# NathanBWaters/playaid_core

Measured on AMD Instinct MI355X. Metric: 1080p frames/sec end-to-end, higher is better.
Workload: dtype f32; 1 GPU; configs[1]: 64 x 1080x1920 BGR frames per GPU per clip; parallelism=single GPU, lanes=2, ingest=raw BGR frames resident in HBM

## Files before the change

include/playaid_hip.h:

```cpp
#ifndef PLAYAID_HIP_H
#define PLAYAID_HIP_H

#include <stddef.h>
#include <stdint.h>

#ifdef __cplusplus
extern "C" {
#endif

#define PA_ABI_VERSION 15
#define PA_WEIGHT_MAGIC 0x31574150
#define PA_LSTM_MAGIC 0x314c4150
#define PA_ENCODER_MAGIC 0x31454150
#define PA_FEATURE_STRIDE 1024
#define PA_CROP 128

typedef enum pa_status {
    PA_OK = 0,
    PA_ERR_INVALID_ARG = -1,
    PA_ERR_HIP = -2,
    PA_ERR_BAD_WEIGHTS = -3,
    PA_ERR_CAPACITY = -4,
    PA_ERR_NO_DEVICE = -5,
    PA_ERR_NOT_READY = -6,
// ... 312 lines not shown
int pa_wino_transform_weights(const float* w_host, int32_t cin, int32_t cout, int32_t bn, float* ug_host);
int pa_wino_conv3x3(const float* x, const float* ug, const float* bias, const float* residual, float* out, int32_t n,
                    int32_t height, int32_t width, int32_t cin, int32_t cout, int32_t bn, int32_t in_px_stride,
                    int32_t out_px_stride, int32_t out_pad, int32_t act, int32_t res_after, void* stream);
int pa_wino_conv3x3_splitk(const float* x, const float* ug, const float* bias, const float* residual, float* out, int32_t n,
                           int32_t height, int32_t width, int32_t cin, int32_t cout, int32_t bn, int32_t in_px_stride, int32_t out_px_stride,
                           int32_t out_pad, int32_t act, int32_t res_after, float* slab, size_t slab_floats, int32_t* tickets,
                           int32_t n_tickets, void* stream);

size_t pa_conv_weight_bytes(int32_t cin, int32_t cout, int32_t ksize, int32_t compute_dtype, int32_t has_residual);
int pa_conv_pack_weights(const float* w_host, int32_t cin, int32_t cout, int32_t ksize, int32_t compute_dtype, int32_t has_residual,
                         void* out_host);
int pa_conv2d(const float* x, const void* w, const float* bias, const float* residual, float* out, int32_t n, int32_t height,
              int32_t width, int32_t cin, int32_t cout, int32_t ksize, int32_t stride, int32_t in_pad, int32_t in_px_stride,
              int32_t out_px_stride, int32_t out_pad, int32_t act, int32_t res_after, int32_t compute_dtype, void* stream);

typedef struct pa_encoder pa_encoder;
size_t pa_encoder_blob_bytes(int32_t in_dim, int32_t hidden_dim, int32_t slots, int32_t enc_dim, int32_t num_layers,
                             int32_t ff_dim, int32_t num_actions);
int pa_encoder_create(int32_t device, int32_t in_dim, int32_t hidden_dim, int32_t slots, int32_t enc_dim, int32_t num_heads,
                      int32_t num_layers, int32_t ff_dim, int32_t num_actions, int32_t max_rows, const void* blob_host,
                      size_t blob_bytes, pa_encoder** out);
void pa_encoder_destroy(pa_encoder* h);
const char* pa_encoder_last_error(const pa_encoder* h);
int pa_encoder_forward(pa_encoder* h, const float* feats, int32_t ld, int32_t seq_len, int32_t batch, float* logp, void* stream);


int pa_profile_enable(pa_engine* e, int32_t on);
int pa_profile_read(pa_engine* e, pa_kernel_stat* stats, int32_t max_stats, int32_t* n_stats);

// ... 48 lines not shown
```

playaid_core_amd/_lib.py:

```python
from __future__ import annotations

import ctypes as C
import os

HERE = os.path.dirname(os.path.abspath(__file__))
LIB_PATH = os.environ.get("PA_LIB_PATH") or os.path.join(HERE, "libplayaid_hip.so")

PA_ABI_VERSION = 15
PA_DTYPE_F32 = 0
PA_DTYPE_BF16 = 1
PA_DTYPE_EMULATED_F32 = 2
DTYPES = {"f32": PA_DTYPE_F32, "bf16": PA_DTYPE_BF16, "emulated_f32": PA_DTYPE_EMULATED_F32}
PA_WEIGHT_MAGIC = 0x31574150
PA_LSTM_MAGIC = 0x314C4150
PA_ENCODER_MAGIC = 0x31454150
PA_FEATURE_STRIDE = 1024
PA_TRACE_STAGES = 20
DET_FORMS = ("not_run", "stem_direct", "stem_bf16", "wino", "patch", "pgemm", "pgemm_up", "psgemm", "psgemm_up", "igemm", "sppf",
             "maxpool", "upsample", "absorbed", "decode", "bgemm", "bgemm_up")
CN_FORMS = ("not_run", "stem_pool", "avgpool", "wino", "patch", "igemm_128x128", "igemm_128x64", "igemm_64x64", "psgemm",
            "bgemm", "bgemm_splitk", "avgpool_bf16")
LSTM_FORMS = ("not_run", "steps", "u1", "u2", "u4", "u8", "mfma")

PA_OK = 0
# ... 165 lines not shown
    ("pa_convnet_destroy", None, [_P]),
    ("pa_convnet_last_error", C.c_char_p, [_P]),
    ("pa_convnet_forward", C.c_int, [_P, _P, C.c_int32, _P, C.c_int32, _P]),
    ("pa_convnet_trace", C.c_int, [_P, _P, C.c_int32, C.c_int32, C.c_int32, _P, C.c_size_t, _P]),
    ("pa_convnet_layer_forms", C.c_int, [_P, _P, C.c_int32]),
    ("pa_detector_plan", C.c_int, [_P] * 5 + [C.c_int32] + [_P] * 7),
    ("pa_detector_plan_desc", C.c_int, [_P, _P, _P, C.c_int32, C.c_int32, C.c_longlong, _P, C.c_int32, C.c_longlong, _P]),
    ("pa_square_crops_src", C.c_int, [_P, _P, C.c_int32, C.c_int32, C.c_int32, _P, _P, C.c_int32, C.c_int32, C.c_int32, _P, _P, _P]),
    ("pa_wino_weight_floats", C.c_size_t, [C.c_int32, C.c_int32]),
    ("pa_wino_channels_per_workgroup", C.c_int, [C.c_int32, C.c_int64]),
    ("pa_wino_transform_weights", C.c_int, [_P, C.c_int32, C.c_int32, C.c_int32, _P]),
    ("pa_wino_conv3x3", C.c_int, [_P, _P, _P, _P, _P] + [C.c_int32] * 11 + [_P]),
    ("pa_conv_weight_bytes", C.c_size_t, [C.c_int32] * 5),
    ("pa_conv_pack_weights", C.c_int, [_P] + [C.c_int32] * 5 + [_P]),
    ("pa_conv2d", C.c_int, [_P, _P, _P, _P, _P] + [C.c_int32] * 14 + [_P]),
    ("pa_wino_conv3x3_splitk", C.c_int, [_P, _P, _P, _P, _P] + [C.c_int32] * 11 + [_P, C.c_size_t, _P, C.c_int32, _P]),
    ("pa_crop_resize_width", C.c_int, [_P, _P, C.c_int32, C.c_int32, C.c_int32, C.POINTER(C.c_int32), C.c_int32, C.c_int32, _P, C.c_int32,
                                       C.POINTER(C.c_int32), _P]),
    ("pa_encoder_blob_bytes", C.c_size_t, [C.c_int32] * 7),
    ("pa_encoder_create", C.c_int, [C.c_int32] * 10 + [_P, C.c_size_t, C.POINTER(_P)]),
    ("pa_encoder_destroy", None, [_P]),
    ("pa_encoder_last_error", C.c_char_p, [_P]),
    ("pa_encoder_forward", C.c_int, [_P, _P, C.c_int32, C.c_int32, C.c_int32, _P, _P]),
    ("pa_mjpeg_create", C.c_int, [C.c_int32, C.c_int32, C.c_int32, C.c_int32, C.c_size_t, C.POINTER(_P)]),
    ("pa_mjpeg_destroy", None, [_P]),
    ("pa_mjpeg_last_error", C.c_char_p, [_P]),
    ("pa_mjpeg_probe", C.c_int, [_P, C.c_size_t, C.POINTER(C.c_int32), C.c_char_p, C.c_size_t]),
    ("pa_mjpeg_set_sync_rounds", C.c_int, [_P, C.c_int32]),
    ("pa_mjpeg_set_groups", C.c_int, [_P, C.c_int32]),
    ("pa_mjpeg_last_sync_rounds", C.c_int, [_P]),
# ... 56 lines not shown
```

playaid_core_amd/conv.py:

```python
from __future__ import annotations

import ctypes as C

import numpy as np
import torch

from . import _lib


def pack_weights(w_oihw: np.ndarray, compute_dtype: str = "emulated_f32", has_residual: bool = False) -> np.ndarray:
    lib = _lib.load()
    w = np.ascontiguousarray(np.asarray(w_oihw, dtype=np.float32).transpose(0, 2, 3, 1))
    cout, k, _, cin = w.shape
    dt = _lib.DTYPES[compute_dtype]
    nbytes = lib.pa_conv_weight_bytes(cin, cout, k, dt, int(has_residual))
    if nbytes == 0:
        raise ValueError("cin and cout must be multiples of 32, the kernel 1x1 or 3x3, the dtype 'f32' or 'emulated_f32'")
    out = np.empty(nbytes, dtype=np.uint8)
    rc = lib.pa_conv_pack_weights(w.ctypes.data_as(C.c_void_p), cin, cout, k, dt, int(has_residual), out.ctypes.data_as(C.c_void_p))
    if rc:
        raise ValueError(f"pa_conv_pack_weights: status {rc}")
    return out


# ... 5 lines not shown
        raise ValueError("x_pad: contiguous float32[n, H + 2 pad, W + 2 pad, C] on the device")
    in_pad = (ksize - 1) // 2 if in_pad is None else in_pad
    n, hp, wp, cs = x_pad.shape
    h, w = hp - 2 * in_pad, wp - 2 * in_pad
    oh, ow = h // stride, w // stride
    ops = out_px_stride or cout
    if out is None:
        out = torch.zeros((n, oh + 2 * out_pad, ow + 2 * out_pad, ops), dtype=torch.float32, device=x_pad.device)
    ptr = lambda t_: C.c_void_p(t_.data_ptr()) if t_ is not None else C.c_void_p(0)
    stream = C.c_void_p(torch.cuda.current_stream(x_pad.device).cuda_stream)
    rc = lib.pa_conv2d(ptr(x_pad), ptr(w_packed), ptr(bias), ptr(residual), ptr(out), n, h, w, cin, cout, ksize, stride, in_pad, cs, out.shape[3],
                       out_pad, int(act), int(bool(res_after)), _lib.DTYPES[compute_dtype], stream)
    if rc:
        raise ValueError(f"pa_conv2d: status {rc}")
    return out
```

playaid_core_amd/csrc/conv_rows.hip:

```cpp
#include "conv_rows.h"
#include "../../include/playaid_hip.h"

namespace pa {

GemmParams conv_row_params(const ConvRow& r) {
    const int oh = r.in_h / r.stride, ow = r.in_w / r.stride;
    const int in_hb = r.in_h + 2 * r.in_pad, in_wb = r.in_w + 2 * r.in_pad;
    const int out_hb = oh + 2 * r.out_pad, out_wb = ow + 2 * r.out_pad;
    GemmParams p;
    memset(&p, 0, sizeof(p));
    p.M = r.images * oh * ow;
    p.N = r.cout;
    p.taps = r.ksize * r.ksize;
    p.kw_taps = r.ksize;
    p.chunk = r.cin;
    p.ktot = p.taps * p.chunk;
    p.howo = oh * ow;
    p.wo = ow;
    p.in_px_stride = r.in_px_stride;
    p.in_row_stride = in_wb * r.in_px_stride;
    p.in_img_stride = in_hb * in_wb * r.in_px_stride;
    p.stride = r.stride;
    p.off_y = p.off_x = r.in_pad - (r.ksize - 1) / 2;
    p.out_px_stride = r.out_px_stride;
// ... 119 lines not shown
    if ((long long)n * in_hb * in_wb * in_px_stride >= (1ll << 29) || (long long)n * out_hb * out_wb * out_px_stride >= (1ll << 29)) return PA_ERR_CAPACITY;
    pa::GemmParams p = pa::conv_row_params({ n,  height, width, in_pad, in_px_stride,  cin, cout, ksize, stride,
                                             out_pad, out_px_stride,  act, res_after});
    p.act = x;
    p.wgt = static_cast<const float*>(w);
    p.bias = bias;
    p.residual = residual;
    p.out = out;
    hipError_t e;
    if (compute_dtype == PA_DTYPE_EMULATED_F32) e = pa::launch_psgemm(p, static_cast<const unsigned short*>(w), (size_t)n * p.out_img_stride, 0, static_cast<hipStream_t>(stream));
    else if (residual) return PA_ERR_INVALID_ARG;
    else e = pa::launch_pgemm(p, 0, static_cast<hipStream_t>(stream));
    return e == hipSuccess ? PA_OK : (e == hipErrorInvalidValue ? PA_ERR_INVALID_ARG : PA_ERR_HIP);
}

}
```

playaid_core_amd/csrc/pa_api.hip:

```cpp
#include "../../include/playaid_hip.h"
#include "conv_rows.h"

#include <algorithm>
#include <cmath>
#include <cstdio>
#include <cstdlib>
#include <cstring>
#include <string>
#include <vector>

using namespace pa;

namespace {

constexpr int WINO_TICKETS = 4096;

struct ConvLayer {
    std::string name;
    int cin, cout, kh, kw, stride;
    int in_hw, out_hw;
    int in_pad, out_pad;
    int off;
    int taps, kw_taps, chunk;
    int in_px_stride;
// ... 2 lines not shown
    float* residual = nullptr;
    float* wgt = nullptr;
    float* wino_wgt = nullptr;
    int wino_bn = 0;
    float* bias = nullptr;
    int relu = 1;
    GemmTile tile = TILE_128x64;
    int splitk = 1;
    bool forced = false;
    float* in2 = nullptr;
    int in2_c = 0, in2_hw = 0, in2_stride = 1;
    float* ds_wgt = nullptr;
    float* ds_out = nullptr;
    float* ds_next_wgt = nullptr;
    float* ds_next_out = nullptr;
    bool ds_fused = false;
    bool ds_probe = false;
    double k_alg = 0;
    unsigned short* split_wgt = nullptr;
    unsigned short* ds_split_wgt = nullptr;
};

struct ProfEntry {
    int name_id;
    hipEvent_t start, stop;
    double flops, bytes;
    double flops_executed;
};

}
// ... 274 lines not shown
    p.ktot = L.taps * L.chunk;
    p.skip_w = L.kh == 7;
    p.howo = L.out_hw * L.out_hw;
    p.wo = L.out_hw;
    p.in_px_stride = L.in_px_stride;
    p.in_row_stride = in_w * L.in_px_stride;
    p.in_img_stride = (int)in_crop;
    p.stride = L.stride;
    p.off_y = L.off;
    p.off_x = L.off;
    p.out_px_stride = L.cout;
    p.out_row_stride = out_w * L.cout;
    p.out_img_stride = (int)out_crop;
    p.out_pad = L.out_pad;
    p.relu = L.relu;
    auto branch_gemm = [&]() {
        GemmParams d = conv_row_params({ ncrops,  L.in2_hw, L.in2_hw, 1, L.in2_c,
                                         L.in2_c, L.cout, 1, L.in2_stride,
                                         L.out_pad, L.cout,  0, 0});
        d.act = at(L.in2, (size_t)crop0 * (L.in2_hw + 2) * (L.in2_hw + 2) * L.in2_c);
        d.wgt = L.ds_wgt;
        d.out = at(L.ds_out, crop0 * out_crop);
        d.slab = p.slab;
        return d;
    };
    if (bf_ds && L.ds_fused) {
        p.residual = at(L.ds_out, crop0 * out_crop);
    } else if (bf_ds) {
        const GemmParams d = branch_gemm();
        ProfScope ps(e, s, prof_name, 2.0 * d.M * d.N * L.in2_c,
                     2.0 * ((double)ncrops * L.in2_hw * L.in2_hw * L.in2_c / (L.in2_stride * L.in2_stride) + (double)d.M * d.N + (double)d.N * L.in2_c));
        HIPCHK(e, launch_igemm_bf16(d, TILE_128x64, s));
        p.residual = d.out;
    } else if (f32_ds) {
        const GemmParams d = branch_gemm();
        ProfScope ps(e, s, prof_name, ds_done ? 0.0 : 2.0 * d.M * d.N * L.in2_c,
                     ds_done ? 0.0 : 4.0 * ((double)ncrops * L.in2_hw * L.in2_hw * L.in2_c / (L.in2_stride * L.in2_stride) + (double)d.M * d.N + (double)d.N * L.in2_c));
        if (ds_done) {
        } else if (e->emu && L.ds_split_wgt) {
            HIPCHK(e, launch_psgemm(d, L.ds_split_wgt, (size_t)ncrops * out_crop, 0, s));
        } else {
            GemmTile dt;
            int dsk;
            choose_tile(d.M, d.N, L.in2_c / 32, &dt, &dsk);
            HIPCHK(e, launch_igemm(d, dt, s));
        }
        if (ds_only) return PA_OK;
        p.residual = d.out;
    } else if (L.in2) {
        const int w2 = L.in2_hw + 2;
        p.act2 = at(L.in2, (size_t)crop0 * w2 * w2 * L.in2_c);
        p.k2_steps = L.in2_c / (bf ? 64 : 32);
        p.in2_px_stride = L.in2_c;
        p.in2_row_stride = w2 * L.in2_c;
        p.in2_img_stride = w2 * w2 * L.in2_c;
        p.stride2 = L.in2_stride;
        p.off2 = 1;
        p.ktot += L.in2_c;
    }
    GemmTile tile = L.tile;
    int splitk = L.splitk;
    if (!L.forced) choose_tile(p.M, p.N, p.ktot / (bf ? 64 : 32), &tile, &splitk);
    p.splitk = splitk;
    const size_t slab_avail = e->slab_floats > slab_off ? e->slab_floats - slab_off : 0;
    if ((size_t)p.splitk * p.M * p.N > slab_avail) p.splitk = 1;
    const bool ds_here = bf && L.ds_next_wgt;
    if (ds_here) {
        p.wgt2 = L.ds_next_wgt;
        p.out2 = at(L.ds_next_out, crop0 * out_crop);
    }
    if (ds_here || (bf && L.ds_probe)) {
        tile = (p.N % 128 == 0 && ((p.M + 127) / 128) * (p.N / 128) >= 256) ? TILE_128x128 : TILE_128x64;
        p.splitk = 1;
    }
    const double k_main = ((bf_ds || f32_ds) ? L.k_alg - L.in2_c : L.k_alg) + (ds_here ? L.cin : 0);
    const double flops = 2.0 * p.M * p.N * k_main;
    const double bytes = (double)es * ((double)ncrops * L.in_hw * L.in_hw * L.cin + (double)p.M * p.N * ((L.residual || bf_ds || f32_ds || ds_here) ? 2 : 1) +
                                       (double)p.N * k_main + ((L.in2 && !bf_ds && !f32_ds) ? (double)ncrops * L.in2_hw * L.in2_hw * L.in2_c : 0.0));
    const bool as_wino = !bf && L.wino_wgt && !p.act2;
    ProfScope ps(e, s, prof_name, flops, bytes, as_wino ? flops * 4.0 / 9.0 : flops);
    static const int use_patch = getenv("PA_PATCH") ? atoi(getenv("PA_PATCH")) : 1;
    static const int use_bf16_patch = getenv("PA_BF16_PATCH") ? atoi(getenv("PA_BF16_PATCH")) : 1;
    if (e->emu && L.split_wgt && !p.act2 && !p.residual) {
        HIPCHK(e, launch_psgemm(p, L.split_wgt, (size_t)ncrops * out_crop, 0, s));
    } else if (bf) {
        hipError_t pe = hipErrorInvalidValue;
        if (use_bf16_patch && L.stride == 1 && !p.act2) pe = launch_conv3x3_bf16_patch(p, s);
        if (pe == hipErrorInvalidValue) {
            static const int t256 = getenv("PA_BF16_T256") ? atoi(getenv("PA_BF16_T256")) : 1;
            if (t256 && !p.out2 && tile == TILE_128x128 && p.splitk == 1 && ((p.M + 255) / 256) * (p.N / 128) >= 256) tile = TILE_256x128;
            pe = launch_igemm_bf16(p, tile, s);
        }
        HIPCHK(e, pe);
    } else if (L.wino_wgt && !p.act2) {
        WinoParams q = wino_params(p, ncrops, L.out_hw, L.out_hw, L.cin, L.wino_wgt, L.wino_bn);
        if (e->wino_tickets && e->slab) {
            q.slab = e->slab + slab_off;
            q.slab_floats = e->slab_floats > slab_off ? std::min(e->slab_floats - slab_off, e->slab_floats / 2) : 0;
            q.tickets = reinterpret_cast<int32_t*>(e->wino_tickets) + (slab_off ? WINO_TICKETS : 0);
            q.tickets_cap = WINO_TICKETS;
        }
        HIPCHK(e, launch_wino3x3(q, s));
    } else if (use_patch && L.kh == 3 && L.stride == 1) {
        int bm = tile == TILE_64x64 || tile == TILE_64x64_K64 ? 64 : 128;
        const int howo = L.out_hw * L.out_hw, in_w2 = L.out_hw + 2;
        const int px128 = howo >= 128 ? (128 / L.out_hw + 2) * in_w2 : (128 / howo) * in_w2 * in_w2;
        if (bm == 128 && px128 > 224) bm = 64;
        hipError_t pe = launch_conv3x3_patch(p, bm, s);
        if (pe == hipErrorInvalidValue) pe = launch_igemm(p, tile, s);
        HIPCHK(e, pe);
    } else {
        static const int use_pgemm = getenv("PA_S2_PGEMM") ? atoi(getenv("PA_S2_PGEMM")) : 2;
        hipError_t pe = hipErrorInvalidValue;
        if (use_pgemm && L.kh == 3 && L.stride == 2 && !p.act2 && !p.residual && p.splitk <= 1 && !p.gather) pe = launch_pgemm(p, use_pgemm == 2 ? 64 : 0, s);
        if (pe == hipErrorInvalidValue) pe = launch_igemm(p, tile, s);
        HIPCHK(e, pe);
    }
    return PA_OK;
}

int run_backbone_part(pa_engine* e, int crop0, int ncrops, const float* x_in, float* feats_out, size_t slab_off, hipStream_t s,
                      int stop = PA_TRACE_STAGES) {
    int rc;
    ConvLayer stem = e->convs[0];
    stem.in = const_cast<float*>(x_in);
    static const bool stem_igemm = getenv("PA_STEM_IGEMM") && atoi(getenv("PA_STEM_IGEMM"));
    auto stem_part = [&](int c0, int n, hipStream_t st) -> int {
        if (stem_igemm && !e->bf16) return run_conv(e, stem, c0, n, slab_off, st, "igemm_conv7x7_stem");
        StemParams sp;
        memset(&sp, 0, sizeof(sp));
        sp.x = x_in + (size_t)c0 * 134 * 134 * 4;
// ... 436 lines not shown
                    rc = upload(e, &L.wgt, wf);
                    if (rc) return rc;
                    static const int wino_mode = getenv("PA_WINO") ? atoi(getenv("PA_WINO")) : 1;
                    static const int wino_ds = getenv("PA_WINO_DS") ? atoi(getenv("PA_WINO_DS")) : 1;
                    static const int wino_min_hw = getenv("PA_WINO_MIN_HW") ? atoi(getenv("PA_WINO_MIN_HW")) : 4;
                    if (wino_mode && wino_ds && hw_out >= wino_min_hw && hw_out % 4 == 0) {
                        L.wino_bn = wino_pick_bn(co, (long long)NC * (hw_out / 4) * (hw_out / 4), co);
                        std::vector<float> ug(wino_weight_floats(co, co), 0.f);
                        if (!br.dry) wino_transform_weights(keep_w.data(), co, co, L.wino_bn, ug.data());
                        rc = upload(e, &L.wino_wgt, ug);
                        if (rc) return rc;
                        rc = upload(e, &L.ds_wgt, wd);
                        if (rc) return rc;
                        if (e->emu && (rc = upload_split(e, &L.ds_split_wgt, wd, co, cin, false))) return rc;
                        ALLOC(L.ds_out, buf, true);
                    }
                }
                rc = upload(e, &L.bias, bf);
                if (rc) return rc;
                L.in2 = cur;
                L.in2_c = cin;
                L.in2_hw = hw_in[li];
                L.in2_stride = stride;
                L.k_alg += cin;
            }
            rc = add_conv(pre + ".1.conv1", co, co, 3, 1, hw_out, outA, mid, nullptr, 1);
            if (rc) return rc;
            rc = add_conv(pre + ".1.conv2", co, co, 3, 1, hw_out, mid, outB, outA, 1);
            if (rc) return rc;
            cur = outB;
// ... 999 lines not shown
```

playaid_core_amd/csrc/pigemm.hip:

```cpp
#include "pgemm_common.h"

#include <algorithm>
#include <type_traits>
#include <cstdio>
#include <cstdlib>
#include <vector>

namespace pa {


namespace {

typedef __attribute__((address_space(3))) float lds_f32;
typedef __attribute__((address_space(3))) f32x4 lds_f32x4;

template <int N> __device__ __forceinline__ void pg_wait_vm() { wait_vmcnt<(N > 63 ? 63 : N)>(); }

}

template <int BM, int BN = 64, bool SILU = true, bool STAMP = false, bool UP = false>
__global__ __launch_bounds__(256, 2) void pgemm_kernel(const GemmParams p) {
    auto stamp = [&](int i) {
        if (STAMP) {
            const unsigned long long t = __builtin_amdgcn_s_memtime();
            if ((threadIdx.x & 63) == 0) p.clk[((size_t)blockIdx.x * 4 + (threadIdx.x >> 6)) * 64 + i] = t;
        }
    };
    stamp(0);
    constexpr int WM = BN == 64 ? 2 : 4;
    constexpr int MI = BM / WM / 32;
    constexpr int A_ROWS = BM / 32, B_ROWS = BN / 32;
    constexpr int NLD = A_ROWS + B_ROWS;
    constexpr int NST = MI * 4 * (UP ? 5 : 1);
    constexpr int STAGE = (BM + BN) * 32;
    __shared__ __attribute__((aligned(16))) float lds[3 * STAGE];

    const TileRun run = tile_run(p);
    const int tile_n = run.tile_n, nt = run.nt;
    {
        const float *pa_ = p.act, *pw_ = p.wgt, *pb_ = p.bias;
        float* po_ = p.out;
        const int i0 = p.M, i1 = p.ktot, i2 = p.kw_taps, i3 = p.chunk, i4 = p.howo, i5 = p.wo, i6 = p.in_img_stride, i7 = p.in_row_stride,
                  i8 = p.in_px_stride, i9 = p.stride, i10 = p.off_y, i11 = p.off_x, i12 = p.out_img_stride, i13 = p.out_row_stride,
                  i14 = p.out_px_stride, i15 = p.out_pad, i16 = p.pg_ho, i17 = p.pg_nwx, i18 = p.pg_nwy;
        const unsigned u0 = p.pg_magic_howo, u1 = p.pg_magic_wo;
        asm volatile("" ::"s"(pa_), "s"(pw_), "s"(pb_), "s"(po_), "s"(i0), "s"(i1), "s"(i2), "s"(i3), "s"(i4), "s"(i5), "s"(i6), "s"(i7), "s"(i8), "s"(i9),
                     "s"(i10), "s"(i11), "s"(i12), "s"(i13), "s"(i14), "s"(i15), "s"(i16), "s"(i17), "s"(i18), "s"(u0), "s"(u1));
    }
    if (nt == 0) return;
    stamp(60);
    const int nk = p.ktot >> 5;
    const int total = nt * nk;

    const int tid = threadIdx.x;
    const int wave_id = __builtin_amdgcn_readfirstlane(tid >> 6);
    const int row0 = tid >> 3;
    const int colq = (tid & 7) ^ ((row0 >> 1) & 7);
    const int lane = tid & 63, lr = lane & 31, lh = lane >> 5;
    const int wm = BN == 64 ? wave_id >> 1 : wave_id, wn = BN == 64 ? wave_id & 1 : 0;

    const __amdgpu_buffer_rsrc_t act_rs = glds_rsrc(p.act), wgt_rs = glds_rsrc(p.wgt);

    const int ch0 = tile_n * BN + wn * 32 + 4 * lh;
    f32x2 nl2e = f32x2{-1.44269504088896341f, -1.44269504088896341f}, one2 = f32x2{1.f, 1.f};
    asm volatile("" : "+v"(nl2e), "+v"(one2));

    int b_off[B_ROWS];
#pragma unroll
    for (int i = 0; i < B_ROWS; ++i) b_off[i] = ((tile_n * BN + row0 + 32 * i) * p.ktot + colq * 4) * 4;

    const int in_ps = p.in_px_stride * p.stride * 4, in_rs = p.in_row_stride * p.stride * 4;
    const int in_wrap_x = in_rs - p.wo * in_ps;
    const int in_wrap_y = p.in_img_stride * 4 - p.pg_ho * in_rs;
    const int in_org = (p.off_y * p.in_row_stride + p.off_x * p.in_px_stride) * 4;
    int in_lane = row0 * in_ps + colq * 16;
    asm volatile("" : "+v"(in_lane));
    const PixelGeom geom = pixel_geom(p);
    int in_last;
    {
        int oy, ox;
        in_last = pixel_base(geom, p.M - 1, p.in_img_stride * 4, in_rs, in_ps, oy, ox) + in_org + colq * 16;
    }
    auto in_offset = [&](int m_base) {
        const int off = pixel_walk(geom, m_base, row0, p.in_img_stride * 4, in_rs, in_ps, in_wrap_x, in_wrap_y, in_org + in_lane);
// ... 13 lines not shown
    auto rows_of = [&](int tile_m) {
#pragma unroll
        for (int i = 0; i < A_ROWS; ++i) a_off[i] = in_offset(tile_m * BM + 32 * i);
    };
    rows_of(cur.tile);
    stamp(61);
    auto issue = [&](int slot) {
        float* As_w = lds + slot * STAGE + wave_id * 256;
        float* Bs_w = As_w + BM * 32;
        const int tapoff = cur.tap_offset(p) * 4;
#pragma unroll
        for (int i = 0; i < A_ROWS; ++i) glds16(act_rs, a_off[i], tapoff, As_w + i * 1024);
        const int koff = ((cur.ky * p.kw_taps + cur.kx) * p.chunk + cur.kc) * 4;
#pragma unroll
        for (int i = 0; i < B_ROWS; ++i) glds16(wgt_rs, b_off[i], koff, Bs_w + i * 1024);
        cur.advance(p, nk, run, rows_of);
    };

    unsigned a_k[4], b_k[4];
    {
        const int a_rd = (wm * (BM / WM) + lr) * 32, b_rd = BM * 32 + (wn * 32 + lr) * 32;
        const int swz = (lr >> 1) & 7;
        const unsigned base = (unsigned)(size_t)(lds_f32*)lds;
#pragma unroll
        for (int kk = 0; kk < 4; ++kk) {
            const int ch_ = ((kk * 2 + lh) ^ swz) * 4;
            a_k[kk] = base + (a_rd + ch_) * 4;
            b_k[kk] = base + (b_rd + ch_) * 4;
            asm volatile("" : "+v"(a_k[kk]), "+v"(b_k[kk]));
        }
    }

    issue(0);
    stamp(62);
    if (total > 1) issue(1);
    f32x16 biasv;
#pragma unroll
    for (int g = 0; g < 4; ++g) {
        const f32x4 b4 = p.bias ? *reinterpret_cast<const f32x4*>(p.bias + ch0 + 8 * g) : f32x4{0.f, 0.f, 0.f, 0.f};
        biasv[4 * g] = b4.x; biasv[4 * g + 1] = b4.y; biasv[4 * g + 2] = b4.z; biasv[4 * g + 3] = b4.w;
    }
    asm volatile("" : "+v"(biasv));
    stamp(1);

    f32x16 acc[MI];
    auto kstep = [&](int sb, auto first_c) {
        constexpr bool FIRST = decltype(first_c)::value;
        unsigned ra[4], rb[4];
#pragma unroll
        for (int kk = 0; kk < 4; ++kk) {
            ra[kk] = a_k[kk] + sb;
            rb[kk] = b_k[kk] + sb;
            asm volatile("" : "+v"(ra[kk]), "+v"(rb[kk]));
        }
        f32x4 af[2][MI], bf[2];
#define PG_FRAGS(SET, KK)                                                                                    \
    {                                                                                                        \
        _Pragma("unroll") for (int mi = 0; mi < MI; ++mi)                                                    \
            af[SET][mi] = *(const lds_f32x4*)(size_t)(ra[KK] + mi * 4096);                                   \
        bf[SET] = *(const lds_f32x4*)(size_t)(rb[KK]);                                                       \
    }
        PG_FRAGS(0, 0);
#pragma unroll
        for (int kk = 0; kk < 4; ++kk) {
#pragma unroll
            for (int mi = 0; mi < MI; ++mi) {
                const f32x4 a4 = af[kk & 1][mi], b4 = bf[kk & 1];
                acc[mi] = __builtin_amdgcn_mfma_f32_32x32x2f32(b4.x, a4.x, FIRST && kk == 0 ? biasv : acc[mi], 0, 0, 0);
                acc[mi] = __builtin_amdgcn_mfma_f32_32x32x2f32(b4.y, a4.y, acc[mi], 0, 0, 0);
                if (mi == 0 && kk + 1 < 4) {
                    __builtin_amdgcn_sched_barrier(0);
                    if (kk == 0) { PG_FRAGS(1, 1); } else if (kk == 1) { PG_FRAGS(0, 2); } else { PG_FRAGS(1, 3); }
                    __builtin_amdgcn_sched_barrier(0);
                }
                acc[mi] = __builtin_amdgcn_mfma_f32_32x32x2f32(b4.z, a4.z, acc[mi], 0, 0, 0);
                acc[mi] = __builtin_amdgcn_mfma_f32_32x32x2f32(b4.w, a4.w, acc[mi], 0, 0, 0);
            }
        }
#undef PG_FRAGS
    };

    int slot = 0, g = 0;
    auto pre = [&](int ks, int t) {
        const bool next = g + 1 < total;
        int closed = 0;
        if (ks == 0 && g > 0) closed = 1;
        if ((nk == 1 || ks == 1) && g > 1) ++closed;
        if (next) {
            if (closed == 2) pg_wait_vm<NLD + 2 * NST>();
            else if (closed == 1) pg_wait_vm<NLD + NST>();
            else pg_wait_vm<NLD>();
        } else {
            if (closed == 2) pg_wait_vm<2 * NST>();
            else if (closed == 1) pg_wait_vm<NST>();
            else pg_wait_vm<0>();
        }
        __builtin_amdgcn_s_barrier();
        if (STAMP && ks == 0 && t < 15) stamp(3 + 4 * t);
        const int slot2 = slot == 0 ? 2 : slot - 1;
        if (g + 2 < total) issue(slot2);
        __builtin_amdgcn_sched_barrier(0);
    };
    for (int t = 0; t < nt; ++t) {
        const int tile_m = run.tile(t);
        if (t < 15) stamp(2 + 4 * t);
        pre(0, t);
        kstep(slot * (STAGE * 4), std::true_type{});
        slot = slot == 2 ? 0 : slot + 1;
        ++g;
        for (int ks = 1; ks < nk; ++ks, ++g) {
            pre(ks, t);
            kstep(slot * (STAGE * 4), std::false_type{});
            slot = slot == 2 ? 0 : slot + 1;
        }
        if (t < 15) stamp(4 + 4 * t);
#pragma unroll
        for (int mi = 0; mi < MI; ++mi) {
            const int m_base = tile_m * BM + wm * (BM / WM) + mi * 32;
            float* o_px = p.out + out_offset(m_base);
            const bool live = m_base + lr < p.M;
            f32x4 out4[4];
#pragma unroll
            for (int gq = 0; gq < 4; ++gq) {
                f32x2 lo = f32x2{acc[mi][4 * gq], acc[mi][4 * gq + 1]}, hi = f32x2{acc[mi][4 * gq + 2], acc[mi][4 * gq + 3]};
                if (SILU) {
                    const f32x2 tl = lo * nl2e, th = hi * nl2e;
                    const f32x2 dl = f32x2{__builtin_amdgcn_exp2f(tl.x), __builtin_amdgcn_exp2f(tl.y)} + one2;
                    const f32x2 dh = f32x2{__builtin_amdgcn_exp2f(th.x), __builtin_amdgcn_exp2f(th.y)} + one2;
                    lo *= f32x2{__builtin_amdgcn_rcpf(dl.x), __builtin_amdgcn_rcpf(dl.y)};
                    hi *= f32x2{__builtin_amdgcn_rcpf(dh.x), __builtin_amdgcn_rcpf(dh.y)};
                } else if (p.relu == 1) {
                    lo.x = lo.x > 0.f ? lo.x : 0.f; lo.y = lo.y > 0.f ? lo.y : 0.f;
                    hi.x = hi.x > 0.f ? hi.x : 0.f; hi.y = hi.y > 0.f ? hi.y : 0.f;
                }
                if (live) *reinterpret_cast<f32x4*>(o_px + 8 * gq) = f32x4{lo.x, lo.y, hi.x, hi.y};
                if (UP) { out4[gq] = f32x4{lo.x, lo.y, hi.x, hi.y}; }
            }
            if (UP && live) {
                float* u_px = p.up_out + pixel_walk(geom, m_base, lr, p.up_img_stride, up_rs, up_ps, up_wrap_x, up_wrap_y, up_lane);
#pragma unroll
                for (int q4 = 0; q4 < 4; ++q4) {
                    float* u = u_px + (q4 >> 1) * p.up_row_stride + (q4 & 1) * p.up_px_stride;
#pragma unroll
                    for (int gq = 0; gq < 4; ++gq) *reinterpret_cast<f32x4*>(u + 8 * gq) = out4[gq];
                }
            }
        }
        if (t < 15) stamp(5 + 4 * t);
    }
    stamp(63);
}

hipError_t launch_pgemm(const GemmParams& p_in, int bm, hipStream_t s) {
    GemmParams p = p_in;
    if (p.residual || p.N % 32 != 0 || (bm != 128 && bm != 64 && bm != 0) || persistent_plan(p) != hipSuccess) return hipErrorInvalidValue;
    const int bn = p.N % 64 == 0 ? 64 : 32;
    if (bn == 32) bm = 128;
    p.tiles_n = p.N / bn;
    if (p.tiles_n > 64) return hipErrorInvalidValue;
    auto plan = [&](int bm_, int* lm_out) {
        const int tm = (p.M + bm_ - 1) / bm_, share = (tm + 7) / 8;
        int lm = 64 / p.tiles_n;
        lm = lm < 1 ? 1 : (lm > share ? share : lm);
        *lm_out = lm;
        return (double)((share + lm - 1) / lm) * (bm_ == 128 ? 1.0 : 0.55) * (lm * p.tiles_n <= 32 ? 0.6 : 1.0);
    };
    int lm = 1;
    if (bm == 0) {
        int lm128, lm64;
        const double e128 = plan(128, &lm128), e64 = plan(64, &lm64);
        bm = e128 <= e64 ? 128 : 64;
        lm = bm == 128 ? lm128 : lm64;
    } else {
        (void)plan(bm, &lm);
    }
    p.tiles_m = (p.M + bm - 1) / bm;
    if ((long long)(p.tiles_m - 1) * bm >= p.M || (long long)p.tiles_m * bm < p.M) return hipErrorInvalidValue;
    const int per = lm * p.tiles_n;
    const int grid = per * 8;
    p.pg_per = per;
    const bool silu = p.relu == 2;
    static const char* stamp_file = getenv("PA_PG_STAMP_FILE");
    if (stamp_file && bm == 128 && bn == 64 && silu) {
        static int sm = 0, sk = 0, sn = 0, skip = getenv("PA_PG_STAMP_SKIP") ? atoi(getenv("PA_PG_STAMP_SKIP")) : 3, seen = 0;
        if (!sm && getenv("PA_PG_STAMP_SHAPE")) sscanf(getenv("PA_PG_STAMP_SHAPE"), "%d,%d,%d", &sm, &sk, &sn);
        if (p.M == sm && p.ktot == sk && p.N == sn && seen++ == skip) {
            const size_t n = (size_t)grid * 4 * 64;
            unsigned long long* d = nullptr;
            if (hipMalloc(&d, n * 8) != hipSuccess) return hipErrorOutOfMemory;
            (void)hipMemsetAsync(d, 0, n * 8, s);
            p.clk = d;
            hipLaunchKernelGGL((pgemm_kernel<128, 64, true, true>), dim3(grid), dim3(256), 0, s, p);
            std::vector<unsigned long long> hst(n);
            (void)hipStreamSynchronize(s);
            (void)hipMemcpy(hst.data(), d, n * 8, hipMemcpyDeviceToHost);
            (void)hipFree(d);
            if (FILE* f = fopen(stamp_file, "wb")) {
                const int hdr[4] = {grid, p.ktot / 32, p.tiles_m, p.tiles_n};
                fwrite(hdr, 4, 4, f);
                fwrite(hst.data(), 8, n, f);
                fclose(f);
            }
            return hipGetLastError();
        }
    }
#define PA_PG_LAUNCH(BM_, BN_)                                                                               \
    do {                                                                                                     \
        if (p.up_out) hipLaunchKernelGGL((pgemm_kernel<BM_, BN_, true, false, true>), dim3(grid), dim3(256), 0, s, p); \
        else if (silu) hipLaunchKernelGGL((pgemm_kernel<BM_, BN_, true>), dim3(grid), dim3(256), 0, s, p);   \
        else hipLaunchKernelGGL((pgemm_kernel<BM_, BN_, false>), dim3(grid), dim3(256), 0, s, p);            \
    } while (0)
    if (p.up_out && (!silu || p.up_px_stride % 4 || p.up_row_stride % 4 || p.up_img_stride % 4 || (reinterpret_cast<unsigned long long>(p.up_out) & 15ull)))
        return hipErrorInvalidValue;
    if (bn == 32) PA_PG_LAUNCH(128, 32);
    else if (bm == 128) PA_PG_LAUNCH(128, 64);
    else PA_PG_LAUNCH(64, 64);
#undef PA_PG_LAUNCH
    return hipGetLastError();
}

}
```

Baseline: 63100 frames/s.

## Fuse f32 ResNet downsample 1x1 branch into stride-2 3x3 pgemm kernel

Adds a branch form of the persistent pgemm kernel that computes the 1x1 stride-2 downsample projection alongside the main stride-2 3x3 conv. It reuses the centre-tap activation tiles already staged in LDS and keeps a second accumulator. The f32 path in the engine now wires the downsample layer into the preceding conv and falls back to a separate igemm launch if the fused launch is rejected. This removes a separate kernel launch and a second read of the input activations, at the cost of extra LDS per stage, a doubled accumulator register footprint and forced 64-row tiles.

Measured after the change: 64110 frames/s, median of 6. 1.6% higher.

```diff
diff --git a/include/playaid_hip.h b/include/playaid_hip.h
--- a/include/playaid_hip.h
+++ b/include/playaid_hip.h
@@ -350,6 +350,10 @@
 int pa_conv2d(const float* x, const void* w, const float* bias, const float* residual, float* out, int32_t n, int32_t height,
               int32_t width, int32_t cin, int32_t cout, int32_t ksize, int32_t stride, int32_t in_pad, int32_t in_px_stride,
               int32_t out_px_stride, int32_t out_pad, int32_t act, int32_t res_after, int32_t compute_dtype, void* stream);
+int pa_conv2d_branch(const float* x, const void* w, const float* bias, const float* residual, float* out, const float* w2, float* out2,
+                     int32_t n, int32_t height, int32_t width, int32_t cin, int32_t cout, int32_t ksize, int32_t stride, int32_t in_pad,
+                     int32_t in_px_stride, int32_t out_px_stride, int32_t out_pad, int32_t act, int32_t res_after, int32_t compute_dtype,
+                     void* stream);
 
 typedef struct pa_encoder pa_encoder;
 size_t pa_encoder_blob_bytes(int32_t in_dim, int32_t hidden_dim, int32_t slots, int32_t enc_dim, int32_t num_layers,
diff --git a/playaid_core_amd/_lib.py b/playaid_core_amd/_lib.py
--- a/playaid_core_amd/_lib.py
+++ b/playaid_core_amd/_lib.py
@@ -203,6 +203,7 @@
     ("pa_conv_weight_bytes", C.c_size_t, [C.c_int32] * 5),
     ("pa_conv_pack_weights", C.c_int, [_P] + [C.c_int32] * 5 + [_P]),
     ("pa_conv2d", C.c_int, [_P, _P, _P, _P, _P] + [C.c_int32] * 14 + [_P]),
+    ("pa_conv2d_branch", C.c_int, [_P, _P, _P, _P, _P, _P, _P] + [C.c_int32] * 14 + [_P]),
     ("pa_wino_conv3x3_splitk", C.c_int, [_P, _P, _P, _P, _P] + [C.c_int32] * 11 + [_P, C.c_size_t, _P, C.c_int32, _P]),
     ("pa_crop_resize_width", C.c_int, [_P, _P, C.c_int32, C.c_int32, C.c_int32, C.POINTER(C.c_int32), C.c_int32, C.c_int32, _P, C.c_int32,
                                        C.POINTER(C.c_int32), _P]),
diff --git a/playaid_core_amd/conv.py b/playaid_core_amd/conv.py
--- a/playaid_core_amd/conv.py
+++ b/playaid_core_amd/conv.py
@@ -43,3 +43,25 @@
     if rc:
         raise ValueError(f"pa_conv2d: status {rc}")
     return out
+
+
+def conv2d_branch(x_pad: torch.Tensor, w: torch.Tensor, w2: torch.Tensor, cin: int, cout: int, bias=None, out=None, out2=None, out_pad: int = 0,
+                  act: int = 0, in_pad: int = 1, ksize: int = 3, stride: int = 2, compute_dtype: str = "f32"):
+    lib = _lib.load()
+    if x_pad.dtype != torch.float32 or not x_pad.is_cuda or not x_pad.is_contiguous() or x_pad.dim() != 4:
+        raise ValueError("x_pad: contiguous float32[n, H + 2 pad, W + 2 pad, C] on the device")
+    n, hp, wp, cs = x_pad.shape
+    h, wd = hp - 2 * in_pad, wp - 2 * in_pad
+    oh, ow = h // stride, wd // stride
+    mk = lambda: torch.zeros((n, oh + 2 * out_pad, ow + 2 * out_pad, cout), dtype=torch.float32, device=x_pad.device)
+    out = mk() if out is None else out
+    out2 = mk() if out2 is None else out2
+    if out2.shape != out.shape:
+        raise ValueError("out2 is addressed like out: same shape")
+    ptr = lambda t_: C.c_void_p(t_.data_ptr()) if t_ is not None else C.c_void_p(0)
+    stream = C.c_void_p(torch.cuda.current_stream(x_pad.device).cuda_stream)
+    rc = lib.pa_conv2d_branch(ptr(x_pad), ptr(w), ptr(bias), C.c_void_p(0), ptr(out), ptr(w2), ptr(out2), n, h, wd, cin, cout, ksize, stride, in_pad, cs,
+                              out.shape[3], out_pad, int(act), 0, _lib.DTYPES[compute_dtype], stream)
+    if rc:
+        raise ValueError(f"pa_conv2d_branch: status {rc}")
+    return out, out2
diff --git a/playaid_core_amd/csrc/conv_rows.hip b/playaid_core_amd/csrc/conv_rows.hip
--- a/playaid_core_amd/csrc/conv_rows.hip
+++ b/playaid_core_amd/csrc/conv_rows.hip
@@ -157,4 +157,30 @@
     return e == hipSuccess ? PA_OK : (e == hipErrorInvalidValue ? PA_ERR_INVALID_ARG : PA_ERR_HIP);
 }
 
+int pa_conv2d_branch(const float* x, const void* w, const float* bias, const float* residual, float* out, const float* w2, float* out2, int32_t n,
+                     int32_t height, int32_t width, int32_t cin, int32_t cout, int32_t ksize, int32_t stride, int32_t in_pad, int32_t in_px_stride,
+                     int32_t out_px_stride, int32_t out_pad, int32_t act, int32_t res_after, int32_t compute_dtype, void* stream) {
+    if (!x || !w || !out || !w2 || !out2 || residual || res_after || n <= 0 || height <= 0 || width <= 0 || ksize != 3 || stride != 2 || height % 2 || width % 2 ||
+        in_pad < 1 || in_px_stride != cin || out_px_stride < cout || out_pad < 0 || act < 0 || act > 1 || compute_dtype != PA_DTYPE_F32 ||
+        pa_conv_weight_bytes(cin, cout, 3, compute_dtype, 0) == 0)
+        return PA_ERR_INVALID_ARG;
+    auto misaligned = [](const void* q) { return (reinterpret_cast<unsigned long long>(q) & 15ull) != 0; };
+    if (in_px_stride % 4 || out_px_stride % 4 || misaligned(x) || misaligned(w) || misaligned(out) || misaligned(w2) || misaligned(out2) ||
+        (reinterpret_cast<unsigned long long>(bias) & 3ull))
+        return PA_ERR_INVALID_ARG;
+    const int oh = height / 2, ow = width / 2;
+    const int in_wb = width + 2 * in_pad, in_hb = height + 2 * in_pad, out_wb = ow + 2 * out_pad, out_hb = oh + 2 * out_pad;
+    if ((long long)n * in_hb * in_wb * in_px_stride >= (1ll << 29) || (long long)n * out_hb * out_wb * out_px_stride >= (1ll << 29)) return PA_ERR_CAPACITY;
+    pa::GemmParams p = pa::conv_row_params({ n,  height, width, in_pad, in_px_stride,  cin, cout, 3, 2,
+                                             out_pad, out_px_stride,  act, 0});
+    p.act = x;
+    p.wgt = static_cast<const float*>(w);
+    p.bias = bias;
+    p.out = out;
+    p.wgt2 = w2;
+    p.out2 = out2;
+    const hipError_t e = pa::launch_pgemm(p, 64, static_cast<hipStream_t>(stream));
+    return e == hipSuccess ? PA_OK : (e == hipErrorInvalidValue ? PA_ERR_INVALID_ARG : PA_ERR_HIP);
 }
+
+}
diff --git a/playaid_core_amd/csrc/pa_api.hip b/playaid_core_amd/csrc/pa_api.hip
--- a/playaid_core_amd/csrc/pa_api.hip
+++ b/playaid_core_amd/csrc/pa_api.hip
@@ -40,6 +40,7 @@
     float* ds_out = nullptr;
     float* ds_next_wgt = nullptr;
     float* ds_next_out = nullptr;
+    std::string ds_next_name;
     bool ds_fused = false;
     bool ds_probe = false;
     double k_alg = 0;
@@ -344,17 +345,24 @@
     p.out_img_stride = (int)out_crop;
     p.out_pad = L.out_pad;
     p.relu = L.relu;
-    auto branch_gemm = [&]() {
-        GemmParams d = conv_row_params({ ncrops,  L.in2_hw, L.in2_hw, 1, L.in2_c,
-                                         L.in2_c, L.cout, 1, L.in2_stride,
+    auto branch_gemm_of = [&](float* src, int hw, int c, int stride, float* wgt, float* out) {
+        GemmParams d = conv_row_params({ ncrops,  hw, hw, 1, c,
+                                         c, L.cout, 1, stride,
                                          L.out_pad, L.cout,  0, 0});
-        d.act = at(L.in2, (size_t)crop0 * (L.in2_hw + 2) * (L.in2_hw + 2) * L.in2_c);
-        d.wgt = L.ds_wgt;
-        d.out = at(L.ds_out, crop0 * out_crop);
+        d.act = at(src, (size_t)crop0 * (hw + 2) * (hw + 2) * c);
+        d.wgt = wgt;
+        d.out = at(out, crop0 * out_crop);
         d.slab = p.slab;
         return d;
     };
-    if (bf_ds && L.ds_fused) {
+    auto branch_gemm = [&]() { return branch_gemm_of(L.in2, L.in2_hw, L.in2_c, L.in2_stride, L.ds_wgt, L.ds_out); };
+    auto launch_f32_branch = [&](const GemmParams& d) {
+        GemmTile dt;
+        int dsk;
+        choose_tile(d.M, d.N, d.chunk / 32, &dt, &dsk);
+        return launch_igemm(d, dt, s);
+    };
+    if ((bf_ds || f32_ds) && L.ds_fused) {
         p.residual = at(L.ds_out, crop0 * out_crop);
     } else if (bf_ds) {
         const GemmParams d = branch_gemm();
@@ -370,10 +378,7 @@
         } else if (e->emu && L.ds_split_wgt) {
             HIPCHK(e, launch_psgemm(d, L.ds_split_wgt, (size_t)ncrops * out_crop, 0, s));
         } else {
-            GemmTile dt;
-            int dsk;
-            choose_tile(d.M, d.N, L.in2_c / 32, &dt, &dsk);
-            HIPCHK(e, launch_igemm(d, dt, s));
+            HIPCHK(e, launch_f32_branch(d));
         }
         if (ds_only) return PA_OK;
         p.residual = d.out;
@@ -394,12 +399,14 @@
     p.splitk = splitk;
     const size_t slab_avail = e->slab_floats > slab_off ? e->slab_floats - slab_off : 0;
     if ((size_t)p.splitk * p.M * p.N > slab_avail) p.splitk = 1;
-    const bool ds_here = bf && L.ds_next_wgt;
-    if (ds_here) {
+    const bool f32_branch = !bf && !e->emu && L.ds_next_wgt;
+    const bool f32_branch_here = f32_branch && p.splitk <= 1;
+    const bool ds_here = (bf && L.ds_next_wgt) || f32_branch_here;
+    if (bf && L.ds_next_wgt) {
         p.wgt2 = L.ds_next_wgt;
         p.out2 = at(L.ds_next_out, crop0 * out_crop);
     }
-    if (ds_here || (bf && L.ds_probe)) {
+    if ((bf && L.ds_next_wgt) || (bf && L.ds_probe)) {
         tile = (p.N % 128 == 0 && ((p.M + 127) / 128) * (p.N / 128) >= 256) ? TILE_128x128 : TILE_128x64;
         p.splitk = 1;
     }
@@ -408,43 +415,61 @@
     const double bytes = (double)es * ((double)ncrops * L.in_hw * L.in_hw * L.cin + (double)p.M * p.N * ((L.residual || bf_ds || f32_ds || ds_here) ? 2 : 1) +
                                        (double)p.N * k_main + ((L.in2 && !bf_ds && !f32_ds) ? (double)ncrops * L.in2_hw * L.in2_hw * L.in2_c : 0.0));
     const bool as_wino = !bf && L.wino_wgt && !p.act2;
-    ProfScope ps(e, s, prof_name, flops, bytes, as_wino ? flops * 4.0 / 9.0 : flops);
-    static const int use_patch = getenv("PA_PATCH") ? atoi(getenv("PA_PATCH")) : 1;
-    static const int use_bf16_patch = getenv("PA_BF16_PATCH") ? atoi(getenv("PA_BF16_PATCH")) : 1;
-    if (e->emu && L.split_wgt && !p.act2 && !p.residual) {
-        HIPCHK(e, launch_psgemm(p, L.split_wgt, (size_t)ncrops * out_crop, 0, s));
-    } else if (bf) {
-        hipError_t pe = hipErrorInvalidValue;
-        if (use_bf16_patch && L.stride == 1 && !p.act2) pe = launch_conv3x3_bf16_patch(p, s);
-        if (pe == hipErrorInvalidValue) {
-            static const int t256 = getenv("PA_BF16_T256") ? atoi(getenv("PA_BF16_T256")) : 1;
-            if (t256 && !p.out2 && tile == TILE_128x128 && p.splitk == 1 && ((p.M + 255) / 256) * (p.N / 128) >= 256) tile = TILE_256x128;
-            pe = launch_igemm_bf16(p, tile, s);
-        }
-        HIPCHK(e, pe);
-    } else if (L.wino_wgt && !p.act2) {
-        WinoParams q = wino_params(p, ncrops, L.out_hw, L.out_hw, L.cin, L.wino_wgt, L.wino_bn);
-        if (e->wino_tickets && e->slab) {
-            q.slab = e->slab + slab_off;
-            q.slab_floats = e->slab_floats > slab_off ? std::min(e->slab_floats - slab_off, e->slab_floats / 2) : 0;
-            q.tickets = reinterpret_cast<int32_t*>(e->wino_tickets) + (slab_off ? WINO_TICKETS : 0);
-            q.tickets_cap = WINO_TICKETS;
-        }
-        HIPCHK(e, launch_wino3x3(q, s));
-    } else if (use_patch && L.kh == 3 && L.stride == 1) {
-        int bm = tile == TILE_64x64 || tile == TILE_64x64_K64 ? 64 : 128;
-        const int howo = L.out_hw * L.out_hw, in_w2 = L.out_hw + 2;
-        const int px128 = howo >= 128 ? (128 / L.out_hw + 2) * in_w2 : (128 / howo) * in_w2 * in_w2;
-        if (bm == 128 && px128 > 224) bm = 64;
-        hipError_t pe = launch_conv3x3_patch(p, bm, s);
-        if (pe == hipErrorInvalidValue) pe = launch_igemm(p, tile, s);
-        HIPCHK(e, pe);
-    } else {
-        static const int use_pgemm = getenv("PA_S2_PGEMM") ? atoi(getenv("PA_S2_PGEMM")) : 2;
-        hipError_t pe = hipErrorInvalidValue;
-        if (use_pgemm && L.kh == 3 && L.stride == 2 && !p.act2 && !p.residual && p.splitk <= 1 && !p.gather) pe = launch_pgemm(p, use_pgemm == 2 ? 64 : 0, s);
-        if (pe == hipErrorInvalidValue) pe = launch_igemm(p, tile, s);
-        HIPCHK(e, pe);
+    bool branch_left = f32_branch;
+    {
+        ProfScope ps(e, s, prof_name, flops, bytes, as_wino ? flops * 4.0 / 9.0 : flops);
+        static const int use_patch = getenv("PA_PATCH") ? atoi(getenv("PA_PATCH")) : 1;
+        static const int use_bf16_patch = getenv("PA_BF16_PATCH") ? atoi(getenv("PA_BF16_PATCH")) : 1;
+        if (e->emu && L.split_wgt && !p.act2 && !p.residual) {
+            HIPCHK(e, launch_psgemm(p, L.split_wgt, (size_t)ncrops * out_crop, 0, s));
+        } else if (bf) {
+            hipError_t pe = hipErrorInvalidValue;
+            if (use_bf16_patch && L.stride == 1 && !p.act2) pe = launch_conv3x3_bf16_patch(p, s);
+            if (pe == hipErrorInvalidValue) {
+                static const int t256 = getenv("PA_BF16_T256") ? atoi(getenv("PA_BF16_T256")) : 1;
+                if (t256 && !p.out2 && tile == TILE_128x128 && p.splitk == 1 && ((p.M + 255) / 256) * (p.N / 128) >= 256) tile = TILE_256x128;
+                pe = launch_igemm_bf16(p, tile, s);
+            }
+            HIPCHK(e, pe);
+        } else if (L.wino_wgt && !p.act2) {
+            WinoParams q = wino_params(p, ncrops, L.out_hw, L.out_hw, L.cin, L.wino_wgt, L.wino_bn);
+            if (e->wino_tickets && e->slab) {
+                q.slab = e->slab + slab_off;
+                q.slab_floats = e->slab_floats > slab_off ? std::min(e->slab_floats - slab_off, e->slab_floats / 2) : 0;
+                q.tickets = reinterpret_cast<int32_t*>(e->wino_tickets) + (slab_off ? WINO_TICKETS : 0);
+                q.tickets_cap = WINO_TICKETS;
+            }
+            HIPCHK(e, launch_wino3x3(q, s));
+        } else if (use_patch && L.kh == 3 && L.stride == 1) {
+            int bm = tile == TILE_64x64 || tile == TILE_64x64_K64 ? 64 : 128;
+            const int howo = L.out_hw * L.out_hw, in_w2 = L.out_hw + 2;
+            const int px128 = howo >= 128 ? (128 / L.out_hw + 2) * in_w2 : (128 / howo) * in_w2 * in_w2;
+            if (bm == 128 && px128 > 224) bm = 64;
+            hipError_t pe = launch_conv3x3_patch(p, bm, s);
+            if (pe == hipErrorInvalidValue) pe = launch_igemm(p, tile, s);
+            HIPCHK(e, pe);
+        } else {
+            static const int use_pgemm = getenv("PA_S2_PGEMM") ? atoi(getenv("PA_S2_PGEMM")) : 2;
+            hipError_t pe = hipErrorInvalidValue;
+            const bool pg = use_pgemm && L.kh == 3 && L.stride == 2 && !p.act2 && !p.residual && p.splitk <= 1 && !p.gather;
+            if (pg && f32_branch_here) {
+                p.wgt2 = L.ds_next_wgt;
+                p.out2 = at(L.ds_next_out, crop0 * out_crop);
+                pe = launch_pgemm(p, 64, s);
+                if (pe == hipSuccess) branch_left = false;
+                p.wgt2 = nullptr;
+                p.out2 = nullptr;
+            }
+            if (pg && pe == hipErrorInvalidValue) pe = launch_pgemm(p, use_pgemm == 2 ? 64 : 0, s);
+            if (pe == hipErrorInvalidValue) pe = launch_igemm(p, tile, s);
+            HIPCHK(e, pe);
+        }
+    }
+    if (branch_left) {
+        const GemmParams d = branch_gemm_of(L.in, L.in_hw, L.cin, L.stride, L.ds_next_wgt, L.ds_next_out);
+        ProfScope ps(e, s, e->profile_layers ? L.ds_next_name.c_str() : prof_name, 2.0 * d.M * d.N * L.cin,
+                     4.0 * ((double)ncrops * L.in_hw * L.in_hw * L.cin / (L.stride * L.stride) + (double)d.M * d.N + (double)d.N * L.cin));
+        HIPCHK(e, launch_f32_branch(d));
     }
     return PA_OK;
 }
@@ -911,6 +936,18 @@
                         if (rc) return rc;
                         if (e->emu && (rc = upload_split(e, &L.ds_split_wgt, wd, co, cin, false))) return rc;
                         ALLOC(L.ds_out, buf, true);
+                        static const int f32_ds_fuse = getenv("PA_F32_DS_FUSE") ? atoi(getenv("PA_F32_DS_FUSE")) : 1;
+                        static const int ds_side_knob = getenv("PA_DS_SIDE") ? atoi(getenv("PA_DS_SIDE")) : 0;
+                        static const int s2_pgemm_knob = getenv("PA_S2_PGEMM") ? atoi(getenv("PA_S2_PGEMM")) : 2;
+                        ConvLayer& C1 = e->convs[e->convs.size() - 2];
+                        if (f32_ds_fuse && !ds_side_knob && s2_pgemm_knob && !e->emu && li < 3 && C1.in == cur && C1.kh == 3 &&
+                            C1.stride == 2 && C1.cout == co && C1.out_hw == hw_out && C1.out_pad == L.out_pad && C1.chunk == cin && C1.cin == cin &&
+                            C1.in_hw == hw_in[li] && C1.in_pad == 1 && !C1.forced) {
+                            C1.ds_next_wgt = L.ds_wgt;
+                            C1.ds_next_out = L.ds_out;
+                            C1.ds_next_name = L.name;
+                            L.ds_fused = true;
+                        }
                     }
                 }
                 rc = upload(e, &L.bias, bf);
diff --git a/playaid_core_amd/csrc/pigemm.hip b/playaid_core_amd/csrc/pigemm.hip
--- a/playaid_core_amd/csrc/pigemm.hip
+++ b/playaid_core_amd/csrc/pigemm.hip
@@ -18,8 +18,9 @@
 
 }
 
-template <int BM, int BN = 64, bool SILU = true, bool STAMP = false, bool UP = false>
-__global__ __launch_bounds__(256, 2) void pgemm_kernel(const GemmParams p) {
+template <int BM, int BN, bool SILU, bool STAMP, bool UP, bool DS>
+__device__ __forceinline__ void pgemm_body(const GemmParams& p) {
+    static_assert(!DS || (!UP && !STAMP && !SILU), "the branch form is the ResNet openers': ReLU, no up-sampled copy");
     auto stamp = [&](int i) {
         if (STAMP) {
             const unsigned long long t = __builtin_amdgcn_s_memtime();
@@ -31,8 +32,8 @@
     constexpr int MI = BM / WM / 32;
     constexpr int A_ROWS = BM / 32, B_ROWS = BN / 32;
     constexpr int NLD = A_ROWS + B_ROWS;
-    constexpr int NST = MI * 4 * (UP ? 5 : 1);
-    constexpr int STAGE = (BM + BN) * 32;
+    constexpr int NST = MI * 4 * (UP ? 5 : (DS ? 2 : 1));
+    constexpr int STAGE = (BM + BN + (DS ? BN : 0)) * 32;
     __shared__ __attribute__((aligned(16))) float lds[3 * STAGE];
 
     const TileRun run = tile_run(p);
@@ -46,11 +47,18 @@
         const unsigned u0 = p.pg_magic_howo, u1 = p.pg_magic_wo;
         asm volatile("" ::"s"(pa_), "s"(pw_), "s"(pb_), "s"(po_), "s"(i0), "s"(i1), "s"(i2), "s"(i3), "s"(i4), "s"(i5), "s"(i6), "s"(i7), "s"(i8), "s"(i9),
                      "s"(i10), "s"(i11), "s"(i12), "s"(i13), "s"(i14), "s"(i15), "s"(i16), "s"(i17), "s"(i18), "s"(u0), "s"(u1));
+        if (DS) {
+            const float* pw2_ = p.wgt2;
+            float* po2_ = p.out2;
+            asm volatile("" ::"s"(pw2_), "s"(po2_));
+        }
     }
     if (nt == 0) return;
     stamp(60);
     const int nk = p.ktot >> 5;
     const int total = nt * nk;
+    const int nkc = p.chunk >> 5;
+    const int c_lo = 4 * nkc, c_hi = 5 * nkc;
 
     const int tid = threadIdx.x;
     const int wave_id = __builtin_amdgcn_readfirstlane(tid >> 6);
@@ -60,6 +68,7 @@
     const int wm = BN == 64 ? wave_id >> 1 : wave_id, wn = BN == 64 ? wave_id & 1 : 0;
 
     const __amdgpu_buffer_rsrc_t act_rs = glds_rsrc(p.act), wgt_rs = glds_rsrc(p.wgt);
+    const __amdgpu_buffer_rsrc_t wgt2_rs = glds_rsrc(DS ? p.wgt2 : p.wgt);
 
     const int ch0 = tile_n * BN + wn * 32 + 4 * lh;
     f32x2 nl2e = f32x2{-1.44269504088896341f, -1.44269504088896341f}, one2 = f32x2{1.f, 1.f};
@@ -68,6 +77,9 @@
     int b_off[B_ROWS];
 #pragma unroll
     for (int i = 0; i < B_ROWS; ++i) b_off[i] = ((tile_n * BN + row0 + 32 * i) * p.ktot + colq * 4) * 4;
+    int b2_off[B_ROWS];
+#pragma unroll
+    for (int i = 0; i < B_ROWS; ++i) b2_off[i] = DS ? ((tile_n * BN + row0 + 32 * i) * p.chunk + colq * 4) * 4 : 0;
 
     const int in_ps = p.in_px_stride * p.stride * 4, in_rs = p.in_row_stride * p.stride * 4;
     const int in_wrap_x = in_rs - p.wo * in_ps;
@@ -111,6 +123,10 @@
         const int koff = ((cur.ky * p.kw_taps + cur.kx) * p.chunk + cur.kc) * 4;
 #pragma unroll
         for (int i = 0; i < B_ROWS; ++i) glds16(wgt_rs, b_off[i], koff, Bs_w + i * 1024);
+        if (DS && cur.ky == 1 && cur.kx == 1) {
+#pragma unroll
+            for (int i = 0; i < B_ROWS; ++i) glds16(wgt2_rs, b2_off[i], cur.kc * 4, Bs_w + BN * 32 + i * 1024);
+        }
         cur.advance(p, nk, run, rows_of);
     };
 
@@ -141,8 +157,16 @@
     stamp(1);
 
     f32x16 acc[MI];
-    auto kstep = [&](int sb, auto first_c) {
+    f32x16 acc2[MI];
+    auto kstep = [&](int sb, auto first_c, auto branch_c) {
         constexpr bool FIRST = decltype(first_c)::value;
+        constexpr int BR = decltype(branch_c)::value;
+        f32x16 zero16;
+        if (BR == 1) {
+#pragma unroll
+            for (int e = 0; e < 16; ++e) zero16[e] = 0.f;
+        }
+        f32x4 b2f[2];
         unsigned ra[4], rb[4];
 #pragma unroll
         for (int kk = 0; kk < 4; ++kk) {
@@ -156,6 +180,7 @@
         _Pragma("unroll") for (int mi = 0; mi < MI; ++mi)                                                    \
             af[SET][mi] = *(const lds_f32x4*)(size_t)(ra[KK] + mi * 4096);                                   \
         bf[SET] = *(const lds_f32x4*)(size_t)(rb[KK]);                                                       \
+        if (BR) b2f[SET] = *(const lds_f32x4*)(size_t)(rb[KK] + BN * 128);                                    \
     }
         PG_FRAGS(0, 0);
 #pragma unroll
@@ -172,6 +197,13 @@
                 }
                 acc[mi] = __builtin_amdgcn_mfma_f32_32x32x2f32(b4.z, a4.z, acc[mi], 0, 0, 0);
                 acc[mi] = __builtin_amdgcn_mfma_f32_32x32x2f32(b4.w, a4.w, acc[mi], 0, 0, 0);
+                if (BR) {
+                    const f32x4 c4 = b2f[kk & 1];
+                    acc2[mi] = __builtin_amdgcn_mfma_f32_32x32x2f32(c4.x, a4.x, BR == 1 && kk == 0 ? zero16 : acc2[mi], 0, 0, 0);
+                    acc2[mi] = __builtin_amdgcn_mfma_f32_32x32x2f32(c4.y, a4.y, acc2[mi], 0, 0, 0);
+                    acc2[mi] = __builtin_amdgcn_mfma_f32_32x32x2f32(c4.z, a4.z, acc2[mi], 0, 0, 0);
+                    acc2[mi] = __builtin_amdgcn_mfma_f32_32x32x2f32(c4.w, a4.w, acc2[mi], 0, 0, 0);
+                }
             }
         }
 #undef PG_FRAGS
@@ -202,19 +234,22 @@
         const int tile_m = run.tile(t);
         if (t < 15) stamp(2 + 4 * t);
         pre(0, t);
-        kstep(slot * (STAGE * 4), std::true_type{});
+        kstep(slot * (STAGE * 4), std::true_type{}, std::integral_constant<int, 0>{});
         slot = slot == 2 ? 0 : slot + 1;
         ++g;
         for (int ks = 1; ks < nk; ++ks, ++g) {
             pre(ks, t);
-            kstep(slot * (STAGE * 4), std::false_type{});
+            if (DS && ks == c_lo) kstep(slot * (STAGE * 4), std::false_type{}, std::integral_constant<int, 1>{});
+            else if (DS && ks > c_lo && ks < c_hi) kstep(slot * (STAGE * 4), std::false_type{}, std::integral_constant<int, 2>{});
+            else kstep(slot * (STAGE * 4), std::false_type{}, std::integral_constant<int, 0>{});
             slot = slot == 2 ? 0 : slot + 1;
         }
         if (t < 15) stamp(4 + 4 * t);
 #pragma unroll
         for (int mi = 0; mi < MI; ++mi) {
             const int m_base = tile_m * BM + wm * (BM / WM) + mi * 32;
-            float* o_px = p.out + out_offset(m_base);
+            const int o_off = out_offset(m_base);
+            float* o_px = p.out + o_off;
             const bool live = m_base + lr < p.M;
             f32x4 out4[4];
 #pragma unroll
@@ -233,6 +268,12 @@
                 if (live) *reinterpret_cast<f32x4*>(o_px + 8 * gq) = f32x4{lo.x, lo.y, hi.x, hi.y};
                 if (UP) { out4[gq] = f32x4{lo.x, lo.y, hi.x, hi.y}; }
             }
+            if (DS && live) {
+                float* o2_px = p.out2 + o_off;
+#pragma unroll
+                for (int gq = 0; gq < 4; ++gq)
+                    *reinterpret_cast<f32x4*>(o2_px + 8 * gq) = f32x4{acc2[mi][4 * gq], acc2[mi][4 * gq + 1], acc2[mi][4 * gq + 2], acc2[mi][4 * gq + 3]};
+            }
             if (UP && live) {
                 float* u_px = p.up_out + pixel_walk(geom, m_base, lr, p.up_img_stride, up_rs, up_ps, up_wrap_x, up_wrap_y, up_lane);
 #pragma unroll
@@ -246,11 +287,27 @@
         if (t < 15) stamp(5 + 4 * t);
     }
     stamp(63);
+}
+
+template <int BM, int BN = 64, bool SILU = true, bool STAMP = false, bool UP = false>
+__global__ __launch_bounds__(256, 2) void pgemm_kernel(const GemmParams p) {
+    pgemm_body<BM, BN, SILU, STAMP, UP, false>(p);
+}
+
+__global__ __launch_bounds__(256, 2) void pgemm_branch_kernel(const GemmParams p) {
+    pgemm_body<64, 64, false, false, false, true>(p);
 }
 
 hipError_t launch_pgemm(const GemmParams& p_in, int bm, hipStream_t s) {
     GemmParams p = p_in;
     if (p.residual || p.N % 32 != 0 || (bm != 128 && bm != 64 && bm != 0) || persistent_plan(p) != hipSuccess) return hipErrorInvalidValue;
+    const bool branch = p.wgt2 || p.out2;
+    if (branch) {
+        if (!p.wgt2 || !p.out2 || p.taps != 9 || p.kw_taps != 3 || p.stride != 2 || p.in_px_stride != p.chunk || p.splitk > 1 || p.N % 64 != 0 || p.relu == 2 || p.up_out ||
+            ((reinterpret_cast<unsigned long long>(p.wgt2) | reinterpret_cast<unsigned long long>(p.out2)) & 15ull))
+            return hipErrorInvalidValue;
+        bm = 64;
+    }
     const int bn = p.N % 64 == 0 ? 64 : 32;
     if (bn == 32) bm = 128;
     p.tiles_n = p.N / bn;
@@ -278,7 +335,7 @@
     p.pg_per = per;
     const bool silu = p.relu == 2;
     static const char* stamp_file = getenv("PA_PG_STAMP_FILE");
-    if (stamp_file && bm == 128 && bn == 64 && silu) {
+    if (stamp_file && bm == 128 && bn == 64 && silu && !branch) {
         static int sm = 0, sk = 0, sn = 0, skip = getenv("PA_PG_STAMP_SKIP") ? atoi(getenv("PA_PG_STAMP_SKIP")) : 3, seen = 0;
         if (!sm && getenv("PA_PG_STAMP_SHAPE")) sscanf(getenv("PA_PG_STAMP_SHAPE"), "%d,%d,%d", &sm, &sk, &sn);
         if (p.M == sm && p.ktot == sk && p.N == sn && seen++ == skip) {
@@ -309,7 +366,8 @@
     } while (0)
     if (p.up_out && (!silu || p.up_px_stride % 4 || p.up_row_stride % 4 || p.up_img_stride % 4 || (reinterpret_cast<unsigned long long>(p.up_out) & 15ull)))
         return hipErrorInvalidValue;
-    if (bn == 32) PA_PG_LAUNCH(128, 32);
+    if (branch) hipLaunchKernelGGL(pgemm_branch_kernel, dim3(grid), dim3(256), 0, s, p);
+    else if (bn == 32) PA_PG_LAUNCH(128, 32);
     else if (bm == 128) PA_PG_LAUNCH(128, 64);
     else PA_PG_LAUNCH(64, 64);
 #undef PA_PG_LAUNCH
```
